# BlaineHeffron/WaveformML

Measured on AMD Instinct MI355X. Metric: waveforms/sec (LitPSD sparse-conv training step), higher is better.
Workload: dtype bf16; 1 GPU; SubMConv3d PSD net, 14x11 PMT grid x 256 samples, Cin=2 Cout=32, 256 events/rank/step, rulebook rebuilt every step; active_voxels_per_rank=84164, global_batch=256, parallelism=dp1, execution=hipgraph

## Files before the change

### include/wfsparse.h

```cpp
#ifndef WFSPARSE_H
#define WFSPARSE_H

#include <stddef.h>
#include <stdint.h>

#ifdef __cplusplus
extern "C" {
#endif

#define WFS_OK 0
#define WFS_EINVAL 1
#define WFS_EOVERFLOW 2
#define WFS_EHIP 3
#define WFS_EWORKSPACE 4

#define WFS_F32 0
#define WFS_BF16 1
#define WFS_F16 2

#define WFS_MAX_DIM 4

#define WFS_ABI_VERSION 6
int wfs_abi_version(void);
const char *wfs_last_error(void);
// ... 188 lines not shown
int wfs_tcnc_ok(int32_t c0, const int32_t *channels, int32_t levels, int32_t k, int32_t L, int32_t dtype);
int wfs_tcnc_n_conv(int32_t c0, const int32_t *channels, int32_t levels, int32_t k);
size_t wfs_tcnc_weights_floats(int32_t c0, const int32_t *channels, int32_t levels, int32_t k);
size_t wfs_tcnc_saved_floats(int64_t N, int32_t L, int32_t c0, const int32_t *channels, int32_t levels);
size_t wfs_tcnc_bwd_workspace_floats(int64_t N, int32_t L, int32_t c0, const int32_t *channels, int32_t levels,
                                     int32_t k);
int wfs_tcnc_taps_fwd(const void *param_ptrs, int32_t c0, const int32_t *channels, int32_t levels, int32_t k,
                      float *wts, void *stream);
int wfs_tcnc_fwd(const void *X, int64_t N, int32_t L, int32_t c0, const int32_t *channels, int32_t levels, int32_t k,
                 const float *wts, float *saved, void *Y, int32_t dtype, float dropout_p, const int64_t *seed_dev,
                 void *stream);
int wfs_tcnc_bwd(const void *X, const void *dY, int64_t N, int32_t L, int32_t c0, const int32_t *channels,
                 int32_t levels, int32_t k, const float *wts, const float *saved, void *dX, float *workspace,
                 const void *param_ptrs, int32_t dtype, float dropout_p, const int64_t *seed_dev, void *stream);

#define WFS_VOXELIZE_MAX_SAMPLES 4096
size_t wfs_voxelize_offsets_ints(int64_t n_cap, int32_t T);
int wfs_voxelize_plan(const void *rows, const int32_t *coords, int64_t n_cap, int32_t T, const int64_t *n_dev,
                      float threshold, int32_t batch_size, int64_t V_cap, int32_t *row_offsets, int64_t *v_dev,
                      int32_t *event_offsets, int32_t *overflow_dev, int32_t dtype, void *stream);
int wfs_voxelize_emit(const void *rows, const void *values, const int32_t *coords, int64_t n_cap, int32_t T,
                      float threshold, const int32_t *row_offsets, int64_t V_cap, int32_t *indices, void *feats,
                      int32_t dtype, void *stream);
int wfs_voxelize_bwd(const void *dfeat, const int32_t *indices, const int32_t *row_offsets, int64_t n_cap, int32_t T,
                     int64_t V_cap, void *dY, int32_t dtype, void *stream);

int wfs_xent_mean_fwd_bwd(const float *logits, const int64_t *target, int64_t B, int32_t C,
                          int64_t ignore_index, float *loss, float *dlogits, void *stream);

int wfs_sgd_step(float *param, const float *grad, float *momentum_buf, int64_t n, const float *lr_dev,
                 float momentum, float dampening, float weight_decay, int32_t nesterov, int32_t first_step,
                 void *stream);

#define WFS_ADAM_COEF_FLOATS 16
int wfs_adam_step(float *param, const float *grad, float *exp_avg, float *exp_avg_sq, float *max_exp_avg_sq,
                  int64_t n, const double *hyper_dev, float *step_dev, float *coef_dev, int32_t amsgrad,
                  int32_t maximize, int32_t decoupled, void *stream);

int wfs_load_batch(const int32_t *coords, int64_t n, int32_t cols, const int32_t *perm_host, int32_t *coords_dst,
                   int32_t *indices_dst, const void *feats, void *feats_dst, int64_t feat_bytes,
                   const int64_t *labels, int64_t *labels_dst, int64_t B, int64_t *n_valid_dst,
                   int32_t *event_offsets, int32_t events, void *stream);

#define WFS_TIMER_GATHER_CONV 0
#define WFS_TIMER_GATHER_DW 1
#define WFS_TIMER_RULEBOOK 2
#define WFS_TIMER_CONV_BACKWARD 3
#define WFS_TIMER_COUNT 4
int wfs_timing_enable(int32_t on);
int wfs_timing_read(int32_t timer, double *total_ms, int64_t *launches);

#ifdef __cplusplus
}
#endif
#endif
```

### waveformml_amd/_lib.py

```python
import ctypes
import os

import torch

_HERE = os.path.dirname(os.path.abspath(__file__))
LIB_PATH = os.environ.get("WFS_LIB") or os.path.join(_HERE, "lib", "libwfsparse.so")

WFS_OK, WFS_EINVAL, WFS_EOVERFLOW, WFS_EHIP, WFS_EWORKSPACE = 0, 1, 2, 3, 4
WFS_F32, WFS_BF16, WFS_F16 = 0, 1, 2
WFS_MAX_DIM = 4
WFS_ABI_VERSION = 6
TIMER_GATHER_CONV, TIMER_GATHER_DW, TIMER_RULEBOOK, TIMER_CONV_BACKWARD = 0, 1, 2, 3

c_i32p = ctypes.POINTER(ctypes.c_int32)
c_i64p = ctypes.POINTER(ctypes.c_int64)
_vp, _i32, _i64, _sz = ctypes.c_void_p, ctypes.c_int32, ctypes.c_int64, ctypes.c_size_t


class Geometry(ctypes.Structure):
    _fields_ = [("ndim", _i32), ("batch_size", _i32), ("subm", _i32), ("K", _i32),
                ("spatial", _i32 * WFS_MAX_DIM), ("out_shape", _i32 * WFS_MAX_DIM),
                ("ksize", _i32 * WFS_MAX_DIM), ("stride", _i32 * WFS_MAX_DIM),
                ("padding", _i32 * WFS_MAX_DIM), ("dilation", _i32 * WFS_MAX_DIM),
                ("transposed", _i32), ("output_padding", _i32 * WFS_MAX_DIM)]
# ... 66 lines not shown
    "wfs_sparse_head_workspace_bytes": (_sz, [_i32, _i64, _i32, _i32]),
    "wfs_sparse_head_fwd": (ctypes.c_int, [_vp, _vp, _vp, _i64, _vp, _i32, _i64, _i32, _vp, _vp, _i32, _vp, _i32, _vp, _sz,
                                           _vp]),
    "wfs_sparse_head_bwd": (ctypes.c_int, [_vp, _vp, _vp, _vp, _i64, _vp, _i32, _i64, _i32, _vp, _i32, _vp, _vp, _vp, _i32,
                                           _vp, _sz, ctypes.POINTER(DwJob), _vp]),
    "wfs_head_workspace_bytes": (_sz, [_i64, _i64, _i32]),
    "wfs_head_fwd": (ctypes.c_int, [_vp, _i64, _i64, _vp, _vp, _i32, _vp, _i32, _vp]),
    "wfs_head_bwd": (ctypes.c_int, [_vp, _vp, _i64, _i64, _vp, _i32, _vp, _vp, _vp, _i32, _vp, _sz, ctypes.POINTER(DwJob),
                                    _vp]),
    "wfs_tcn_lds_bytes": (_sz, [_i32, _i32, _i32]),
    "wfs_tcn_taps_fwd": (ctypes.c_int, [_vp, _i32, _i32, _vp, _vp, _vp]),
    "wfs_tcn_taps_bwd": (ctypes.c_int, [_vp, _i32, _i32, _vp, _i64, _vp]),
    "wfs_tcn_fwd": (ctypes.c_int, [_vp, _i64, _i32, _vp, _vp, _i32, _i32, _vp, _i32, ctypes.c_float, _vp, _vp]),
    "wfs_tcn_bwd": (ctypes.c_int, [_vp, _vp, _i64, _i32, _vp, _vp, _i32, _i32, _vp, _vp, _i32, ctypes.c_float, _vp,
                                    _vp]),
    "wfs_tcnc_ok": (ctypes.c_int, [_i32, c_i32p, _i32, _i32, _i32, _i32]),
    "wfs_tcnc_n_conv": (ctypes.c_int, [_i32, c_i32p, _i32, _i32]),
    "wfs_tcnc_weights_floats": (_sz, [_i32, c_i32p, _i32, _i32]),
    "wfs_tcnc_saved_floats": (_sz, [_i64, _i32, _i32, c_i32p, _i32]),
    "wfs_tcnc_bwd_workspace_floats": (_sz, [_i64, _i32, _i32, c_i32p, _i32, _i32]),
    "wfs_tcnc_taps_fwd": (ctypes.c_int, [_vp, _i32, c_i32p, _i32, _i32, _vp, _vp]),
    "wfs_tcnc_fwd": (ctypes.c_int, [_vp, _i64, _i32, _i32, c_i32p, _i32, _i32, _vp, _vp, _vp, _i32, ctypes.c_float, _vp,
                                    _vp]),
    "wfs_tcnc_bwd": (ctypes.c_int, [_vp, _vp, _i64, _i32, _i32, c_i32p, _i32, _i32, _vp, _vp, _vp, _vp, _vp, _i32,
                                    ctypes.c_float, _vp, _vp]),
    "wfs_voxelize_offsets_ints": (_sz, [_i64, _i32]),
    "wfs_voxelize_plan": (ctypes.c_int, [_vp, _vp, _i64, _i32, _vp, ctypes.c_float, _i32, _i64, _vp, _vp, _vp, _vp, _i32,
                                         _vp]),
    "wfs_voxelize_emit": (ctypes.c_int, [_vp, _vp, _vp, _i64, _i32, ctypes.c_float, _vp, _i64, _vp, _vp, _i32, _vp]),
    "wfs_voxelize_bwd": (ctypes.c_int, [_vp, _vp, _vp, _i64, _i32, _i64, _vp, _i32, _vp]),
    "wfs_xent_mean_fwd_bwd": (ctypes.c_int, [_vp, _vp, _i64, _i32, _i64, _vp, _vp, _vp]),
    "wfs_sgd_step": (ctypes.c_int, [_vp, _vp, _vp, _i64, _vp, ctypes.c_float, ctypes.c_float, ctypes.c_float, _i32, _i32,
                                    _vp]),
    "wfs_adam_step": (ctypes.c_int, [_vp, _vp, _vp, _vp, _vp, _i64, _vp, _vp, _vp, _i32, _i32, _i32, _vp]),
    "wfs_load_batch": (ctypes.c_int, [_vp, _i64, _i32, c_i32p, _vp, _vp, _vp, _vp, _i64, _vp, _vp, _i64, _vp, _vp, _i32,
                                      _vp]),
    "wfs_timing_enable": (ctypes.c_int, [_i32]),
    "wfs_timing_read": (ctypes.c_int, [_i32, ctypes.POINTER(ctypes.c_double), c_i64p]),
}

_LIB = None


def load():
    global _LIB
    if _LIB is None:
        if not os.path.exists(LIB_PATH):
            raise ImportError(
                "libwfsparse.so is missing at %s -- build it with `make -C waveformml_amd/csrc` "
                "(or python -c 'import __graft_entry__ as g; g.build()').  There is no CPU fallback." % LIB_PATH)
        lib = ctypes.CDLL(LIB_PATH)
        for name, (res, args) in SIGNATURES.items():
            fn = getattr(lib, name)
            fn.restype, fn.argtypes = res, args
        got = lib.wfs_abi_version()
        if got != WFS_ABI_VERSION:
            raise ImportError("%s has ABI version %d, this binding was written for %d (struct layouts / signatures "
                              "differ): rebuild with `make -C waveformml_amd/csrc`" % (LIB_PATH, got, WFS_ABI_VERSION))
        wide = os.environ.get("WFS_WIDE_MIN_CHANNELS")
        if wide is not None:
            lib.wfs_wide_enable(int(wide))
        _LIB = lib
    return _LIB


def last_error():
# ... 59 lines not shown
```

### waveformml_amd/csrc/conv_mfma.hip

```cpp
#include <stdlib.h>

#include "wfs_common.h"

namespace {

typedef float f32x16 __attribute__((ext_vector_type(16)));
typedef float f32x4 __attribute__((ext_vector_type(4)));
constexpr int F32_GROUP = 4;

struct KMap {
    int v[128];
};

__device__ __forceinline__ long long valid_rows(long long R, const long long *r_dev) {
    long long v = r_dev ? *r_dev : R;
    return v < R ? v : R;
}

__device__ __forceinline__ int packed_entry(int e, int o) { return (e >= 0 && (e & 7) == o) ? (e >> 3) : -1; }
__device__ __forceinline__ void table_row_of(int pk, int k, int *trow, int *osel) {
    const int kq = pk ? k / pk : k;
    *trow = kq;
    *osel = pk ? k - kq * pk : -1;
}
__device__ __forceinline__ int table_value(int e, int osel) { return osel < 0 ? e : packed_entry(e, osel); }

typedef __bf16 bf16x8e __attribute__((ext_vector_type(8)));
typedef float f32x2 __attribute__((ext_vector_type(2)));

__device__ __forceinline__ void split3_bf16(f32x4 x, bool keep, uint2 &p1, uint2 &p2, uint2 &p3) {
    unsigned u[4], v[4], w[4];
#pragma unroll
    for (int i = 0; i < 4; i += 2) {
        const float xa = x[i], xb = x[i + 1];
        u[i] = keep ? __builtin_bit_cast(unsigned, xa) : 0u;
        u[i + 1] = keep ? __builtin_bit_cast(unsigned, xb) : 0u;
        const f32x2 full = {__builtin_bit_cast(float, u[i]), __builtin_bit_cast(float, u[i + 1])};
        const f32x2 top = {__builtin_bit_cast(float, u[i] & 0xFFFF0000u), __builtin_bit_cast(float, u[i + 1] & 0xFFFF0000u)};
        const f32x2 r = full - top;
        const float ra = r[0], rb = r[1];
        v[i] = __builtin_bit_cast(unsigned, ra);
// ... 485 lines not shown
    const long long Rv = valid_rows(R, r_dev);
    for (long long row = (long long)blockIdx.x * 32 + rsub; row < Rv; row += (long long)gridDim.x * 32) {
        f32x4 acc = bv;
        for (int k = 0; k < K; ++k) {
            int nb = (k == identity_k) ? (int)row : table[(long long)kmap.v[k] * R + row];
            if (nb < 0) continue;
            float x0 = wfs_ld(X + (long long)nb * 2), x1 = wfs_ld(X + (long long)nb * 2 + 1);
            f32x4 w0 = *(const f32x4 *)(sW + k * 64 + cq * 4);
            f32x4 w1 = *(const f32x4 *)(sW + k * 64 + 32 + cq * 4);
            acc.x = fmaf(x0, w0.x, acc.x);
            acc.y = fmaf(x0, w0.y, acc.y);
            acc.z = fmaf(x0, w0.z, acc.z);
            acc.w = fmaf(x0, w0.w, acc.w);
            acc.x = fmaf(x1, w1.x, acc.x);
            acc.y = fmaf(x1, w1.y, acc.y);
            acc.z = fmaf(x1, w1.z, acc.z);
            acc.w = fmaf(x1, w1.w, acc.w);
        }
        T *y = Y + row * 32 + cq * 4;
        if constexpr (sizeof(T) == 4) {
            *reinterpret_cast<f32x4 *>(y) = acc;
        } else {
            uint2 pk;
            pk.x = wfs_pack2<T>(acc.x, acc.y);
            pk.y = wfs_pack2<T>(acc.z, acc.w);
            *reinterpret_cast<uint2 *>(y) = pk;
        }
    }
}

constexpr int DW_KG = 4;
constexpr int DW_WAVES = 8;

constexpr int DW_LDS = DW_WAVES * 1024 * 4;
template <typename T>
__device__ __forceinline__ void gdw32_body(float *sRed, int bx, int by, int nbx, const int *__restrict__ table, int pk, int K,
                                           int identity_k, long long Rcap, const long long *__restrict__ r_dev,
                                           const T *__restrict__ S, const T *__restrict__ G, float *__restrict__ part,
                                           int ngroups) {
    const int lane = threadIdx.x & 63, wid = threadIdx.x >> 6;
    const int j = lane & 31, h = lane >> 5;
    const int g = by;
    const long long R = valid_rows(Rcap, r_dev);
    const long long ntiles = (R + 31) >> 5;
    static_assert(sizeof(T) == 4, "fp32 rows");
    const __amdgpu_buffer_rsrc_t rsrcS = __builtin_amdgcn_make_buffer_rsrc((void *)S, 0, (int)(R * 128), 0x00020000);
    const __amdgpu_buffer_rsrc_t rsrcG = __builtin_amdgcn_make_buffer_rsrc((void *)G, 0, 0x7FFFFFFF, 0x00020000);
    const unsigned j4 = (unsigned)j * 4u;
    f32x16 acc[DW_KG];
#pragma unroll
    for (int q = 0; q < DW_KG; ++q)
#pragma unroll
        for (int i = 0; i < 16; ++i) acc[q][i] = 0.f;
    int trw[DW_KG], osel[DW_KG];
#pragma unroll
    for (int q = 0; q < DW_KG; ++q) {
        const int k = g + q * ngroups;
        table_row_of(pk, k < K ? k : K - 1, &trw[q], &osel[q]);
    }
    for (long long tile = bx + (long long)wid * nbx; tile < ntiles; tile += (long long)DW_WAVES * nbx) {
        const long long row0 = tile * 32;
        const long long trow = row0 + j < R ? row0 + j : R - 1;
        int nbv[DW_KG];
#pragma unroll
        for (int q = 0; q < DW_KG; ++q) nbv[q] = table_value(table[(long long)trw[q] * Rcap + trow], osel[q]);
        float a[16];
        {
// ... 703 lines not shown
    wfs_dw_job j[MAX_DW_JOBS];
    int first[MAX_DW_JOBS + 1];
    int n;
};
__global__ void __launch_bounds__(1024) k_slab_reduce_multi(DwJobs jobs) {
    __shared__ float sR[32][32];
    int ji = 0;
    while (ji + 1 < jobs.n && (int)blockIdx.x >= jobs.first[ji + 1]) ++ji;
    const wfs_dw_job &jb = jobs.j[ji];
    const int nsl = jb.nslabs > 64 ? 32 : 8;
    const int groups = 32 / nsl;
    const int row = threadIdx.x >> 5, lane = threadIdx.x & 31;
    const int grp = row / nsl, sl = row % nsl;
    const long long e = ((long long)((int)blockIdx.x - jobs.first[ji]) * groups + grp) * 32 + lane;
    float s = 0.f;
    if (e < jb.per)
        for (long long c = sl; c < jb.nslabs; c += nsl) s += jb.part[c * jb.per + e];
    sR[row][lane] = s;
    __syncthreads();
    if (sl == 0 && e < jb.per) {
        s = 0.f;
        for (int q = 0; q < nsl; ++q) s += sR[grp * nsl + q][lane];
        if (jb.transpose) {
            const long long ab = (long long)jb.A * jb.B;
            const int k = (int)(e / ab), rem = (int)(e % ab);
            const int a = rem / jb.B, b = rem % jb.B;
            jb.dW[((long long)k * jb.B + b) * jb.A + a] = s;
        } else {
            jb.dW[e] = s;
        }
    }
}

__global__ void __launch_bounds__(1024) k_slab_reduce_multi4(DwJobs jobs) {
    __shared__ f32x4 sR4[32][32];
    int ji = 0;
    while (ji + 1 < jobs.n && (int)blockIdx.x >= jobs.first[ji + 1]) ++ji;
    const wfs_dw_job &jb = jobs.j[ji];
    const int nsl = jb.nslabs > 64 ? 32 : 8;
    const int groups = 32 / nsl;
    const int row = threadIdx.x >> 5, lane = threadIdx.x & 31;
    const int grp = row / nsl, sl = row % nsl;
    const long long e = (((long long)((int)blockIdx.x - jobs.first[ji]) * groups + grp) * 32 + lane) * 4;
    f32x4 s = {0.f, 0.f, 0.f, 0.f};
    if (e < jb.per) {
        constexpr int U = 6;
        for (long long c0 = sl; c0 < jb.nslabs; c0 += (long long)nsl * U) {
            f32x4 v[U];
#pragma unroll
            for (int u = 0; u < U; ++u) {
                const long long c = c0 + (long long)u * nsl;
                const long long cc = c < jb.nslabs ? c : sl;
                v[u] = *(const f32x4 *)(jb.part + cc * jb.per + e);
            }
#pragma unroll
            for (int u = 0; u < U; ++u)
                if (c0 + (long long)u * nsl < jb.nslabs) s += v[u];
        }
    }
    sR4[row][lane] = s;
    __syncthreads();
    if (sl == 0 && e < jb.per) {
        s = f32x4{0.f, 0.f, 0.f, 0.f};
        for (int q = 0; q < nsl; ++q) s += sR4[grp * nsl + q][lane];
        if (jb.transpose) {
            const long long ab = (long long)jb.A * jb.B;
#pragma unroll
            for (int i = 0; i < 4; ++i) {
                const long long ei = e + i;
                const int k = (int)(ei / ab), rem = (int)(ei % ab);
                const int a = rem / jb.B, b = rem % jb.B;
                jb.dW[((long long)k * jb.B + b) * jb.A + a] = s[i];
            }
        } else if ((reinterpret_cast<uintptr_t>(jb.dW + e) & 15) == 0) {
            *(f32x4 *)(jb.dW + e) = s;
        } else {
#pragma unroll
            for (int i = 0; i < 4; ++i) jb.dW[e + i] = s[i];
        }
    }
}

}

int wfs_launch_dw_jobs(const wfs_dw_job *jobs, int n, hipStream_t stream) {
    DwJobs dj;
    dj.n = n;
    bool by4 = true;
    for (int i = 0; i < n; ++i)
        by4 = by4 && jobs[i].per % 4 == 0 && ((uintptr_t)jobs[i].part & 15) == 0;
    int blocks = 0;
    for (int i = 0; i < n; ++i) {
        dj.j[i] = jobs[i];
        dj.first[i] = blocks;
        const long long per_block = (jobs[i].nslabs > 64 ? 32 : 128) * (by4 ? 4 : 1);
        blocks += (int)((jobs[i].per + per_block - 1) / per_block);
    }
    dj.first[n] = blocks;
    if (blocks == 0) return WFS_OK;
    if (by4)
        k_slab_reduce_multi4<<<dim3((unsigned)blocks), dim3(1024), 0, stream>>>(dj);
    else
        k_slab_reduce_multi<<<dim3((unsigned)blocks), dim3(1024), 0, stream>>>(dj);
    WFS_LAUNCH_CHECK();
    return WFS_OK;
}

static bool wfs_split_bf16() {
    static const int on = [] {
        const char *e = getenv("WFS_SPLIT_BF16");
        return (e && e[0] == '0') ? 0 : 1;
    }();
    return on != 0;
}

bool wfs_mfma_gconv32_ok(int K) { return K >= 1 && K <= 32; }

template <typename KernelT, typename... Args>
static int launch_big_lds(KernelT kernel, bool *attr_done, dim3 grid, dim3 block, size_t lds, hipStream_t stream,
                          Args... args) {
    if (!*attr_done) {
        WFS_HIP_CHECK(hipFuncSetAttribute((const void *)kernel, hipFuncAttributeMaxDynamicSharedMemorySize, 158 * 1024));
        *attr_done = true;
    }
    kernel<<<grid, block, lds, stream>>>(args...);
    WFS_LAUNCH_CHECK();
    return WFS_OK;
}

static void gconv32_grid(long long R, bool padded, long long *ntiles, int *wpb, long long *nblk, long long *tiles_per_xcd,
                         int max_waves) {
    *ntiles = (R + 31) >> 5;
    const long long expect = padded ? (*ntiles * 7 + 7) / 8 : *ntiles;
    int w = (int)((expect + 255) / 256);
    w = w < 4 ? 4 : (w > max_waves ? max_waves : (w + 3) / 4 * 4);
    long long nb = (expect + w - 1) / w;
    if (nb > 256) nb = 256;
// ... 311 lines not shown
```

### waveformml_amd/csrc/optim.hip

```cpp
#include "wfs_common.h"

namespace {

__global__ void __launch_bounds__(256) k_sgd_step(float *__restrict__ P, const float *__restrict__ G,
                                                  float *__restrict__ M, long long n, const float *__restrict__ lr_dev,
                                                  float momentum, float dampening, float weight_decay, int nesterov,
                                                  int first_step) {
    const float lr = *lr_dev;
    for (long long i = (long long)blockIdx.x * 256 + threadIdx.x; i < n; i += (long long)gridDim.x * 256) {
        float p = P[i];
        float g = G[i];
        if (weight_decay != 0.f) g = fmaf(weight_decay, p, g);
        if (M) {
            float b = first_step ? g : fmaf(1.f - dampening, g, M[i] * momentum);
            M[i] = b;
            g = nesterov ? fmaf(momentum, b, g) : b;
        }
        P[i] = fmaf(-lr, g, p);
    }
}

}

extern "C" int wfs_sgd_step(float *param, const float *grad, float *momentum_buf, int64_t n, const float *lr_dev,
                            float momentum, float dampening, float weight_decay, int32_t nesterov, int32_t first_step,
                            void *stream_) {
    hipStream_t stream = (hipStream_t)stream_;
    if (n == 0) return WFS_OK;
    WFS_REQUIRE(param && grad && lr_dev, WFS_EINVAL, "NULL device pointer");
    WFS_REQUIRE(momentum_buf || momentum == 0.f, WFS_EINVAL, "momentum needs a buffer");
    long long blocks = wfs_cdiv(n, 256);
    if (blocks > 2048) blocks = 2048;
    k_sgd_step<<<dim3((unsigned)blocks), dim3(256), 0, stream>>>(param, grad, momentum != 0.f ? momentum_buf : nullptr, n,
                                                                 lr_dev, momentum, dampening, weight_decay, nesterov,
                                                                 first_step);
    WFS_LAUNCH_CHECK();
    return WFS_OK;
}

namespace {

struct AdamCoef {
    float decay, wd, w1, omw1, b2, omb2, bc2s, eps, neg_step;
    int has_wd;
};
static_assert(sizeof(AdamCoef) <= WFS_ADAM_COEF_FLOATS * sizeof(float), "coefficient workspace");

__global__ void __launch_bounds__(64) k_adam_prologue(const double *__restrict__ hp, float *__restrict__ step,
                                                      AdamCoef *__restrict__ coef) {
    if (threadIdx.x != 0) return;
    const float t = *step + 1.f;
    *step = t;
    const double lr = hp[0], beta1 = hp[1], beta2 = hp[2], eps = hp[3], wd = hp[4];
    AdamCoef c;
    c.has_wd = wd != 0.0;
    c.decay = (float)(1.0 - lr * wd);
    c.wd = (float)wd;
    c.w1 = (float)(1.0 - beta1);
    c.omw1 = 1.f - c.w1;
    c.b2 = (float)beta2;
    c.omb2 = (float)(1.0 - beta2);
    const double bc1 = 1.0 - pow(beta1, (double)t), bc2 = 1.0 - pow(beta2, (double)t);
    c.bc2s = (float)sqrt(bc2);
    c.eps = (float)eps;
    c.neg_step = (float)(-(lr / bc1));
    *coef = c;
}

template <bool AMS>
__device__ __forceinline__ void adam1(float &p, float g, float &m, float &v, float &vm, const AdamCoef &c, int maximize,
// ... 177 lines not shown
```

### waveformml_amd/csrc/wfs_common.h

```cpp
#pragma once
#include <hip/hip_runtime.h>
#include <stdint.h>
#include <stdio.h>

#include "../../include/wfsparse.h"

#define WFS_WAVE 64

void wfs_set_error(const char *fmt, ...);

#define WFS_HIP_CHECK(expr)                                                                  \
    do {                                                                                     \
        hipError_t _e = (expr);                                                              \
        if (_e != hipSuccess) {                                                              \
            wfs_set_error("%s failed: %s (%s:%d)", #expr, hipGetErrorString(_e), __FILE__,   \
                          __LINE__);                                                         \
            return WFS_EHIP;                                                                 \
        }                                                                                    \
    } while (0)

#define WFS_LAUNCH_CHECK() WFS_HIP_CHECK(hipGetLastError())

#define WFS_REQUIRE(cond, code, ...)                                                         \
    do {                                                                                     \
// ... 30 lines not shown
template <>
__device__ __forceinline__ void wfs_unpack2<wfs_bf16>(unsigned w, float &lo, float &hi) {
    lo = __uint_as_float(w << 16);
    hi = __uint_as_float(w & 0xFFFF0000u);
}
template <>
__device__ __forceinline__ void wfs_unpack2<wfs_f16>(unsigned w, float &lo, float &hi) {
    typedef _Float16 h2 __attribute__((ext_vector_type(2)));
    h2 v = __builtin_bit_cast(h2, w);
    lo = (float)v.x;
    hi = (float)v.y;
}
template <typename H>
__device__ __forceinline__ unsigned wfs_pack2(float lo, float hi);
template <>
__device__ __forceinline__ unsigned wfs_pack2<wfs_bf16>(float lo, float hi) {
    wfs_bf16 a, b;
    wfs_st(&a, lo);
    wfs_st(&b, hi);
    return (unsigned)a | ((unsigned)b << 16);
}
template <>
__device__ __forceinline__ unsigned wfs_pack2<wfs_f16>(float lo, float hi) {
    typedef _Float16 h2 __attribute__((ext_vector_type(2)));
    h2 v = {(_Float16)lo, (_Float16)hi};
    return __builtin_bit_cast(unsigned, v);
}
template <typename H>
__device__ __forceinline__ float wfs_round_to(float v) {
    H t;
    wfs_st(&t, v);
    return wfs_ld(&t);
}
static inline bool wfs_dtype_ok(int dtype) { return dtype == WFS_F32 || dtype == WFS_BF16 || dtype == WFS_F16; }

struct WfsTimerScope {
    int timer;
    hipStream_t stream;
    void *rec;
    WfsTimerScope(int timer, hipStream_t stream);
    ~WfsTimerScope();
};

bool wfs_mfma_gconv32_ok(int K);
int wfs_launch_gconv32_f32(const int *table, int mirror, int K, int identity_k, long long R, const long long *r_dev,
                           const float *X, const float *W, int transpose_w, const float *bias, float *Y,
                           hipStream_t stream, int packed_kl = 0);
int wfs_launch_gconv32_h16(const int *table, int mirror, int K, int identity_k, long long R, const long long *r_dev,
                           const void *X, const float *W, int transpose_w, const float *bias, void *Y, int dtype,
                           hipStream_t stream, int packed_kl = 0);
int wfs_launch_gconv_c2c32(const int *table, const int *kmap, int K, int identity_k, long long R,
                           const long long *r_dev, const void *X, const float *W, const float *bias, void *Y, int dtype,
                           hipStream_t stream);
bool wfs_wide_dw_ok(int K, long long R, int Cs, int Cg, int dtype);
size_t wfs_wide_dw_workspace(int K, long long R, int Cs, int Cg, int dtype);
int wfs_launch_wide_dw(const int *table, const int *kmap_host, int K, int identity_k, long long R, const long long *r_dev,
                       const void *S, int Cs, const void *G, long long G_rows, int Cg, int swap, float *dW, int dtype,
                       void *workspace, size_t workspace_bytes, hipStream_t stream);
size_t wfs_dw_fast_workspace(int K, long long R, int Cs, int Cg);
int wfs_launch_gdw32(const int *table, int K, int identity_k, long long R, const long long *r_dev, const void *S,
                     const void *G, int swap, float *dW, float *part, int dtype, wfs_dw_job *defer, hipStream_t stream,
                     int packed_kl = 0);
bool wfs_bwd32_fused_ok(int K, int packed_kl, int dtype);
int wfs_launch_bwd32_h16(const int *table, int packed_kl, int K, int identity_k, long long R, const long long *r_dev,
                         const void *S, const void *G, const float *W, void *dX, int swap, float *dW, float *part, int dtype,
                         wfs_dw_job *defer, hipStream_t stream);
int wfs_launch_gdw_c32c2(const int *table, int mirror, int K, int identity_k, long long R, const long long *r_dev,
                         const void *S, const void *G, int swap, float *dW, float *part, int dtype,
                         wfs_dw_job *defer, hipStream_t stream);
int wfs_launch_dw_jobs(const wfs_dw_job *jobs, int n, hipStream_t stream);
```

### waveformml_amd/psd/graph.py

```python
import contextlib
import gc
import os
import sys

import torch
import torch.distributed as dist

from .. import _lib
from ..spconv import ops
from .voxel import Voxelizer


@contextlib.contextmanager
def _no_gc():
    was = gc.isenabled()
    gc.disable()
    try:
        yield
    finally:
        if was:
            gc.enable()


def _round_up(v, m):
# ... 150 lines not shown
            return
        _lib.check(_lib.load().wfs_event_offsets(_lib.ptr(self.indices), self.indices.shape[0], self.indices.shape[1] - 1,
                                                 self.n_events, _lib.ptr(self.n_valid), _lib.ptr(self.events),
                                                 _lib.stream_ptr()))


class GraphedTrainStep(_CapturedRunner):
    def __init__(self, module, optimizer, reducer, example_batch, headroom=None, granule=None, warmup=2, min_rows=0):
        (coords, feats), labels = example_batch
        headroom, granule = self._headroom_granule(int(coords.shape[0]), int(labels.shape[0]), headroom, granule)
        assert labels.is_cuda
        per_row = bool(getattr(module, "per_row_targets", False)) and labels.shape[0] == coords.shape[0]
        if per_row:
            self.ignore_index = int(getattr(getattr(module, "criterion", None), "ignore_index", -100))
        net = self._static_buffers(module, example_batch, headroom, granule, min_rows, per_row)
        self.optimizer, self.reducer = optimizer, reducer
        dev = coords.device
        if per_row and net is not None and hasattr(net, "batch_size_hint"):
            net.batch_size_hint = self.n_cap
        if (ops.EVENT_LOCAL and self.indices is not None and 1 <= self.n_events <= ops.EVENT_LOCAL_MAX_BATCH
                and hasattr(net, "batch_events")):
            self.events = torch.zeros((int(_lib.load().wfs_event_offsets_ints(self.n_events)),), dtype=torch.int32,
                                      device=dev)
            net.batch_events = (self.coords, self.events)
        self.world = reducer.world
        exchange = bool(getattr(reducer, "exchange", self.world > 1))
        self.in_graph_exchange = (exchange and dist.is_available() and dist.is_initialized()
                                  and dist.get_backend(reducer.group) == "nccl"
                                  and os.environ.get("WFS_GRAPH_EXCHANGE", "1") != "0")
        if self.in_graph_exchange:
            self.in_graph_exchange = _collective_capture_works(reducer.group, dev)
        self.exchange_after = exchange and not self.in_graph_exchange
        self.in_graph_optimizer = not self.exchange_after and steps_in_graph(optimizer)
        self._own_stream(dev)
        self._fresh_flags()
        reducer.reset()
        loss = module.training_step(([coords, feats], labels), 0)
        loss.backward()
        reducer.finish()
        optimizer.step()
        del loss
        own = _round_up(headroom * coords.shape[0], granule)
        factor = headroom if self.n_cap <= own else self.n_cap / max(1.0, float(coords.shape[0]))
        slack = 1.06 if headroom < 1.05 else 1.0
        self._calibrate(factor, slack, granule)
        if self.exchange_after:
            reducer.remove()
        if self.indices is not None:
            net.batch_first_indices = (self.coords, self.indices)
        self._load(example_batch)
        failed, err = 0, None
        try:
            self._warm_and_capture(warmup)
        except Exception as e:
            if not self.in_graph_exchange:
                raise
            failed, err = 1, e
        if self.in_graph_exchange and self.world > 1:
            failed = _agree_max(failed, reducer.group)
        if failed:
            print("[waveformml_amd] in-graph gradient exchange could not be captured on some rank (%s); exchanging "
                  "after the replay" % (("%s: %s" % (type(err).__name__, err)) if err is not None else "another rank"),
                  file=sys.stderr, flush=True)
            torch.cuda.synchronize()
            self.in_graph_exchange, self.exchange_after, self.in_graph_optimizer = False, True, False
            reducer.remove()
            self._warm_and_capture(warmup)
        self._collect_flags()

    def _warm_and_capture(self, warmup):
        for _ in range(warmup):
            self._body()
            if not self.in_graph_optimizer:
                self._after()
        torch.cuda.synchronize()
        self.graph, self.loss = self._capture(self._body)

    def close(self, remove_hooks=True):
        if self.graph is not None and remove_hooks:
            self.reducer.remove()
        super().close()
        self.loss = None

    def _static_batch(self):
        return ([self.coords, self.feats, self.n_valid], self.labels)

    def _body(self):
        self.reducer.reset()
        from ..spconv import functional as Fsp
        loss = self.module.training_step(self._static_batch(), 0)
        Fsp.defer_dw(self.reducer.flat_param is not None)
        try:
            if loss.dtype == torch.float32 and loss.dim() == 0:
                torch.autograd.backward(loss, grad_tensors=Fsp.unit_loss_grad(loss.device))
            else:
                loss.backward()
            if self.in_graph_exchange:
                self.reducer.finish()
            else:
                self.reducer.pack_all()
        finally:
            Fsp.defer_dw(False)
        if self.in_graph_optimizer:
            self.optimizer.step()
        return loss.detach()

    def _after(self):
        if self.exchange_after:
            self.reducer.exchange_packed()
        self.optimizer.step()

    def eager_step(self, batch):
        self.reducer.reset()
        net = getattr(self.module, "model", None)
        hint = getattr(net, "batch_size_hint", None)
        if self.per_row and hint is not None:
            net.batch_size_hint = None
        try:
            loss = self.module.training_step(batch, 0)
        finally:
            if self.per_row and hint is not None:
                net.batch_size_hint = hint
        loss.backward()
        if self.exchange_after:
            self.reducer.pack_all()
            self.reducer.exchange_packed()
        else:
            self.reducer.finish()
        self.optimizer.step()
        return loss.detach()

    def fits_counts(self, rows_max, labels_min, labels_max, rows_ne_labels):
        if self.per_row:
            return rows_max <= self.n_cap and not rows_ne_labels
        return rows_max <= self.n_cap and labels_min == labels_max == int(self.labels.shape[0])

# ... 190 lines not shown
```

### waveformml_amd/psd/optim.py

```python
import torch

from .. import _lib


class FlatSGD(torch.optim.SGD):
    flat_device_step = True

    def _fast_groups(self):
        for g in self.param_groups:
            ps = g["params"]
            if (len(ps) != 1 or not ps[0].is_cuda or ps[0].dtype != torch.float32 or not ps[0].is_contiguous()
                    or g.get("maximize", False) or g.get("differentiable", False)):
                return False
        return True

    def sync_hyperparameters(self):
        for g in self.param_groups:
            dev = g["params"][0].device
            if g.get("_lr_dev") is None or g["_lr_dev"].device != dev:
                g["_lr_dev"] = torch.empty((1,), dtype=torch.float32, device=dev)
                g["_lr_host"] = None
            if g["_lr_host"] != float(g["lr"]):
                g["_lr_dev"].fill_(float(g["lr"]))
                g["_lr_host"] = float(g["lr"])

    def state_dict(self):
        sd = super().state_dict()
        for g in sd["param_groups"]:
            g.pop("_lr_dev", None)
            g.pop("_lr_host", None)
        sd["state"] = {k: {n: v for n, v in st.items() if n != "_fresh"} for k, st in sd["state"].items()}
        return sd

    def mark_fresh(self):
        for g in self.param_groups:
            if g["dampening"] != 0 and g["momentum"] != 0:
                for p in g["params"]:
                    if "momentum_buffer" in self.state.get(p, {}):
                        self.state[p]["_fresh"] = True

    def has_fresh(self):
        return any(st.get("_fresh", False) for st in self.state.values())

    @torch.no_grad()
    def step(self, closure=None):
        if closure is not None or not self._fast_groups():
            return super().step(closure)
        lib = _lib.load()
        self.sync_hyperparameters()
        for g in self.param_groups:
            p = g["params"][0]
            if p.grad is None:
                continue
            grad = p.grad
            if grad.is_sparse or grad.dtype != torch.float32 or not grad.is_contiguous():
                return super().step(closure)
            state = self.state[p]
            buf, first = state.get("momentum_buffer"), False
            if g["momentum"] != 0 and buf is None:
                buf = state["momentum_buffer"] = torch.empty_like(p, memory_format=torch.contiguous_format)
                first = True
            if state.pop("_fresh", False) and not torch.cuda.is_current_stream_capturing():
                first = True
            _lib.check(lib.wfs_sgd_step(_lib.ptr(p), _lib.ptr(grad), _lib.ptr(buf) if g["momentum"] != 0 else None,
                                        p.numel(), _lib.ptr(g["_lr_dev"]), float(g["momentum"]), float(g["dampening"]),
                                        float(g["weight_decay"]), 1 if g["nesterov"] else 0, 1 if first else 0,
                                        _lib.stream_ptr()))
        return None


_ADAM_COEF_FLOATS = 16


class _FlatAdamStep(object):
    flat_device_step = True

    def _fast_groups(self):
        for g in self.param_groups:
            ps = g["params"]
            if (len(ps) != 1 or not ps[0].is_cuda or ps[0].dtype != torch.float32 or not ps[0].is_contiguous()
                    or torch.is_tensor(g["lr"]) or g.get("differentiable", False)):
                return False
        return True

    @staticmethod
    def _hyper(g):
        beta1, beta2 = g["betas"]
        return (float(g["lr"]), float(beta1), float(beta2), float(g["eps"]), float(g["weight_decay"]))

    def sync_hyperparameters(self):
        dev_blocks = self.__dict__.setdefault("_flat_dev", {})
        capturing = torch.cuda.is_available() and torch.cuda.is_current_stream_capturing()
        for i, g in enumerate(self.param_groups):
            dev = g["params"][0].device
            blk = dev_blocks.get(i)
            if blk is None or blk[0].device != dev:
                if capturing:
                    raise RuntimeError("FlatAdam: the first step runs outside a graph capture (it allocates the "
                                       "hyperparameter block)")
                blk = dev_blocks[i] = [torch.empty((5,), dtype=torch.float64, device=dev),
                                       torch.zeros((_ADAM_COEF_FLOATS,), dtype=torch.float32, device=dev), [None] * 5]
# ... 62 lines not shown
```

### waveformml_amd/spconv/functional.py

```python
import ctypes

import torch
from torch.autograd import Function

from .. import _lib

CONV, SUBM, INVERSE = 0, 1, 2

ACCOUNT = None


def _account(kind, table, R, rows_in, c_in, rows_out, c_out, K, cw_in, cw_out, esize):
    if ACCOUNT is None:
        return
    pairs = int((table >= 0).sum().item()) if table is not None else int(R)
    ACCOUNT.append(dict(kind=kind, pairs=pairs,
                        bytes=rows_in * c_in * esize + rows_out * c_out * esize + pairs * 8 + K * cw_in * cw_out * 4,
                        flops=2 * pairs * cw_in * cw_out))


def _features_ok(t):
    if not t.is_cuda:
        raise RuntimeError("waveformml_amd.spconv: features must be on the GPU (there is no CPU path)")
    return t.contiguous()
# ... 128 lines not shown
            off = param.data_ptr() - fp.data_ptr()
            if 0 <= off and off + 4 * param.numel() <= 4 * fp.numel() and off % 4 == 0:
                slot = fg.data_ptr() + off
                if slot in _SLOTS_WRITTEN:
                    flush_deferred_dw()
                    _SHARED_SLOTS.add(slot)
                    break
                if not _SLOTS_WRITTEN:
                    try:
                        torch.autograd.Variable._execution_engine.queue_callback(reset_grad_slots)
                    except RuntimeError:
                        pass
                _SLOTS_WRITTEN.add(slot)
                return fg[off // 4: off // 4 + param.numel()].view(shape)
    return torch.empty(shape, dtype=torch.float32, device=param.device)


_DEFERRED_DW = None
_DEFERRED_SLOTS = set()
_SHARED_SLOTS = set()


def defer_dw(on):
    global _DEFERRED_DW
    _DEFERRED_DW = [] if on else None
    _DEFERRED_SLOTS.clear()
    _SHARED_SLOTS.clear()


def was_deferred(slot_ptr):
    return slot_ptr in _DEFERRED_SLOTS and slot_ptr not in _SHARED_SLOTS


def flush_deferred_dw():
    if not _DEFERRED_DW:
        return
    lib = _lib.load()
    jobs = (_lib.DwJob * len(_DEFERRED_DW))(*[j for (j, _ws) in _DEFERRED_DW])
    for at in range(0, len(_DEFERRED_DW), 16):
        n = min(16, len(_DEFERRED_DW) - at)
        _lib.check(lib.wfs_dw_reduce_jobs(ctypes.cast(ctypes.byref(jobs, at * ctypes.sizeof(_lib.DwJob)),
                                                      ctypes.POINTER(_lib.DwJob)), n, _lib.stream_ptr()))
    for j, _ws in _DEFERRED_DW:
        _DEFERRED_SLOTS.add(int(j.dW))
    del _DEFERRED_DW[:]


def join_side_streams():
    if _PENDING_SIDE:
        cur = torch.cuda.current_stream()
        for ev, _keep in _PENDING_SIDE:
            cur.wait_event(ev)
        del _PENDING_SIDE[:]


def gather_dw(table, K, identity_k, R, S, G, swap, kmap=None, r_dev=None, overlap=False, like=None, packed_kl=0):
    lib = _lib.load()
    Cs, Cg = int(S.shape[1]), int(G.shape[1])
    shape = (K, Cg, Cs) if swap else (K, Cs, Cg)
    in_slot = False
    if like is not None and like.numel() == K * Cs * Cg:
        dW = grad_like(like, shape)
        in_slot = dW._base is not None
    else:
        dW = torch.empty(shape, dtype=torch.float32, device=S.device)
    assert S.dtype == G.dtype and S.shape[0] == R
    assert table is None or (table.dtype == torch.int32 and table.shape == ((K // packed_kl if packed_kl else K), R))
    nbytes = lib.wfs_gather_dw_workspace_bytes(K, R, Cs, Cg)
    ws = torch.empty((max(int(nbytes), 1),), dtype=torch.uint8, device=S.device)

    def launch():
        defer = _DEFERRED_DW is not None and in_slot and not overlap
        job = _lib.DwJob() if defer else None
        _lib.check(lib.wfs_gather_dw(_lib.ptr(table), kmap, K, identity_k, R, _lib.ptr(S), Cs, _lib.ptr(G), G.shape[0],
                                     Cg, 1 if swap else 0, _lib.ptr(dW), _lib.dtype_code(S), _lib.ptr(ws), ws.numel(),
                                     _lib.ptr(r_dev), ctypes.byref(job) if defer else None, packed_kl, _lib.stream_ptr()))
        if defer and job.nslabs > 0:
            _DEFERRED_DW.append((job, ws))
# ... 613 lines not shown
```

Measured before the change: 559,800 events/s.

## Fuse deferred dW slab reduction with the SGD optimizer step

After: 562,700 events/s, median of 4. No clear change (+0.5%).

```diff
diff --git a/include/wfsparse.h b/include/wfsparse.h
--- a/include/wfsparse.h
+++ b/include/wfsparse.h
@@ -244,6 +244,10 @@
                  float momentum, float dampening, float weight_decay, int32_t nesterov, int32_t first_step,
                  void *stream);
 
+int wfs_dw_reduce_jobs_sgd(const wfs_dw_job *jobs, int32_t n_jobs, float *param, const float *grad,
+                           float *momentum_buf, int64_t n, const float *lr_dev, float momentum, float dampening,
+                           float weight_decay, int32_t nesterov, int32_t first_step, void *stream);
+
 #define WFS_ADAM_COEF_FLOATS 16
 int wfs_adam_step(float *param, const float *grad, float *exp_avg, float *exp_avg_sq, float *max_exp_avg_sq,
                   int64_t n, const double *hyper_dev, float *step_dev, float *coef_dev, int32_t amsgrad,
diff --git a/waveformml_amd/_lib.py b/waveformml_amd/_lib.py
--- a/waveformml_amd/_lib.py
+++ b/waveformml_amd/_lib.py
@@ -122,6 +122,8 @@
     "wfs_xent_mean_fwd_bwd": (ctypes.c_int, [_vp, _vp, _i64, _i32, _i64, _vp, _vp, _vp]),
     "wfs_sgd_step": (ctypes.c_int, [_vp, _vp, _vp, _i64, _vp, ctypes.c_float, ctypes.c_float, ctypes.c_float, _i32, _i32,
                                     _vp]),
+    "wfs_dw_reduce_jobs_sgd": (ctypes.c_int, [ctypes.POINTER(DwJob), _i32, _vp, _vp, _vp, _i64, _vp, ctypes.c_float,
+                                              ctypes.c_float, ctypes.c_float, _i32, _i32, _vp]),
     "wfs_adam_step": (ctypes.c_int, [_vp, _vp, _vp, _vp, _vp, _i64, _vp, _vp, _vp, _i32, _i32, _i32, _vp]),
     "wfs_load_batch": (ctypes.c_int, [_vp, _i64, _i32, c_i32p, _vp, _vp, _vp, _vp, _i64, _vp, _vp, _i64, _vp, _vp, _i32,
                                       _vp]),
diff --git a/waveformml_amd/csrc/conv_mfma.hip b/waveformml_amd/csrc/conv_mfma.hip
--- a/waveformml_amd/csrc/conv_mfma.hip
+++ b/waveformml_amd/csrc/conv_mfma.hip
@@ -6,7 +6,6 @@
 
 typedef float f32x16 __attribute__((ext_vector_type(16)));
 typedef float f32x4 __attribute__((ext_vector_type(4)));
-constexpr int F32_GROUP = 4;
 
 struct KMap {
     int v[128];
@@ -558,7 +557,6 @@
 constexpr int DW_KG = 4;
 constexpr int DW_WAVES = 8;
 
-constexpr int DW_LDS = DW_WAVES * 1024 * 4;
 template <typename T>
 __device__ __forceinline__ void gdw32_body(float *sRed, int bx, int by, int nbx, const int *__restrict__ table, int pk, int K,
                                            int identity_k, long long Rcap, const long long *__restrict__ r_dev,
@@ -1328,8 +1326,35 @@
     }
 }
 
-__global__ void __launch_bounds__(1024) k_slab_reduce_multi4(DwJobs jobs) {
-    __shared__ f32x4 sR4[32][32];
+constexpr int MAX_SGD_RANGES = MAX_DW_JOBS + 1;
+struct SgdTail {
+    wfs_sgd_args a;
+    int nrange;
+    long long start[MAX_SGD_RANGES];
+    long long cum[MAX_SGD_RANGES + 1];
+};
+
+template <bool SGD>
+__device__ __forceinline__ void slab_reduce4(const DwJobs &jobs, const SgdTail &sgd, f32x4 (*sR4)[32]) {
+    float lr = 0.f;
+    if (SGD) {
+        lr = *sgd.a.lr_dev;
+        if ((int)blockIdx.x >= jobs.first[jobs.n]) {
+            const long long total = sgd.cum[sgd.nrange];
+            const long long nth = (long long)((int)gridDim.x - jobs.first[jobs.n]) * 1024;
+            for (long long v = (long long)((int)blockIdx.x - jobs.first[jobs.n]) * 1024 + threadIdx.x; v < total; v += nth) {
+                long long i = v;
+#pragma unroll
+                for (int r = 0; r < MAX_SGD_RANGES; ++r)
+                    if (r < sgd.nrange && v >= sgd.cum[r]) i = sgd.start[r] + (v - sgd.cum[r]);
+                float m = (sgd.a.M && !sgd.a.first_step) ? sgd.a.M[i] : 0.f;
+                sgd.a.P[i] = wfs_sgd1(sgd.a.P[i], sgd.a.G[i], m, sgd.a.M != nullptr, lr, sgd.a.momentum, sgd.a.dampening,
+                                      sgd.a.weight_decay, sgd.a.nesterov, sgd.a.first_step);
+                if (sgd.a.M) sgd.a.M[i] = m;
+            }
+            return;
+        }
+    }
     int ji = 0;
     while (ji + 1 < jobs.n && (int)blockIdx.x >= jobs.first[ji + 1]) ++ji;
     const wfs_dw_job &jb = jobs.j[ji];
@@ -1338,6 +1363,27 @@
     const int row = threadIdx.x >> 5, lane = threadIdx.x & 31;
     const int grp = row / nsl, sl = row % nsl;
     const long long e = (((long long)((int)blockIdx.x - jobs.first[ji]) * groups + grp) * 32 + lane) * 4;
+    const bool writer = sl == 0 && e < jb.per;
+    long long at[4] = {e, e + 1, e + 2, e + 3};
+    if (jb.transpose && writer) {
+        const long long ab = (long long)jb.A * jb.B;
+#pragma unroll
+        for (int i = 0; i < 4; ++i) {
+            const long long ei = e + i;
+            const int k = (int)(ei / ab), rem = (int)(ei % ab);
+            const int a = rem / jb.B, b = rem % jb.B;
+            at[i] = ((long long)k * jb.B + b) * jb.A + a;
+        }
+    }
+    float p[4] = {0.f, 0.f, 0.f, 0.f}, m[4] = {0.f, 0.f, 0.f, 0.f};
+    const long long gi = SGD ? jb.dW - sgd.a.G : 0;
+    if (SGD && writer) {
+#pragma unroll
+        for (int i = 0; i < 4; ++i) {
+            p[i] = sgd.a.P[gi + at[i]];
+            if (sgd.a.M && !sgd.a.first_step) m[i] = sgd.a.M[gi + at[i]];
+        }
+    }
     f32x4 s = {0.f, 0.f, 0.f, 0.f};
     if (e < jb.per) {
         constexpr int U = 6;
@@ -1356,35 +1402,41 @@
     }
     sR4[row][lane] = s;
     __syncthreads();
-    if (sl == 0 && e < jb.per) {
+    if (writer) {
         s = f32x4{0.f, 0.f, 0.f, 0.f};
         for (int q = 0; q < nsl; ++q) s += sR4[grp * nsl + q][lane];
         if (jb.transpose) {
-            const long long ab = (long long)jb.A * jb.B;
-#pragma unroll
-            for (int i = 0; i < 4; ++i) {
-                const long long ei = e + i;
-                const int k = (int)(ei / ab), rem = (int)(ei % ab);
-                const int a = rem / jb.B, b = rem % jb.B;
-                jb.dW[((long long)k * jb.B + b) * jb.A + a] = s[i];
-            }
+#pragma unroll
+            for (int i = 0; i < 4; ++i) jb.dW[at[i]] = s[i];
         } else if ((reinterpret_cast<uintptr_t>(jb.dW + e) & 15) == 0) {
             *(f32x4 *)(jb.dW + e) = s;
         } else {
 #pragma unroll
             for (int i = 0; i < 4; ++i) jb.dW[e + i] = s[i];
         }
-    }
-}
-
-}
-
-int wfs_launch_dw_jobs(const wfs_dw_job *jobs, int n, hipStream_t stream) {
-    DwJobs dj;
+        if (SGD) {
+#pragma unroll
+            for (int i = 0; i < 4; ++i) {
+                sgd.a.P[gi + at[i]] = wfs_sgd1(p[i], s[i], m[i], sgd.a.M != nullptr, lr, sgd.a.momentum, sgd.a.dampening,
+                                               sgd.a.weight_decay, sgd.a.nesterov, sgd.a.first_step);
+                if (sgd.a.M) sgd.a.M[gi + at[i]] = m[i];
+            }
+        }
+    }
+}
+
+__global__ void __launch_bounds__(1024) k_slab_reduce_multi4(DwJobs jobs) {
+    __shared__ f32x4 sR4[32][32];
+    slab_reduce4<false>(jobs, SgdTail{}, sR4);
+}
+
+__global__ void __launch_bounds__(1024, 8) k_slab_reduce_sgd4(DwJobs jobs, SgdTail sgd) {
+    __shared__ f32x4 sR4[32][32];
+    slab_reduce4<true>(jobs, sgd, sR4);
+}
+
+int dw_job_blocks(const wfs_dw_job *jobs, int n, bool by4, DwJobs &dj) {
     dj.n = n;
-    bool by4 = true;
-    for (int i = 0; i < n; ++i)
-        by4 = by4 && jobs[i].per % 4 == 0 && ((uintptr_t)jobs[i].part & 15) == 0;
     int blocks = 0;
     for (int i = 0; i < n; ++i) {
         dj.j[i] = jobs[i];
@@ -1393,12 +1445,74 @@
         blocks += (int)((jobs[i].per + per_block - 1) / per_block);
     }
     dj.first[n] = blocks;
+    return blocks;
+}
+
+bool dw_jobs_by4(const wfs_dw_job *jobs, int n) {
+    bool by4 = true;
+    for (int i = 0; i < n; ++i)
+        by4 = by4 && jobs[i].per % 4 == 0 && ((uintptr_t)jobs[i].part & 15) == 0;
+    return by4;
+}
+
+}
+
+int wfs_launch_dw_jobs(const wfs_dw_job *jobs, int n, hipStream_t stream) {
+    DwJobs dj;
+    const bool by4 = dw_jobs_by4(jobs, n);
+    const int blocks = dw_job_blocks(jobs, n, by4, dj);
     if (blocks == 0) return WFS_OK;
     if (by4)
         k_slab_reduce_multi4<<<dim3((unsigned)blocks), dim3(1024), 0, stream>>>(dj);
     else
         k_slab_reduce_multi<<<dim3((unsigned)blocks), dim3(1024), 0, stream>>>(dj);
     WFS_LAUNCH_CHECK();
+    return WFS_OK;
+}
+
+int wfs_launch_dw_jobs_sgd(const wfs_dw_job *jobs, int n, const wfs_sgd_args &sgd, int *fused, hipStream_t stream) {
+    *fused = 0;
+    if (n < 1 || n > MAX_DW_JOBS || sgd.n <= 0 || !dw_jobs_by4(jobs, n)) return WFS_OK;
+    long long lo[MAX_DW_JOBS], hi[MAX_DW_JOBS];
+    for (int i = 0; i < n; ++i) {
+        const uintptr_t d = (uintptr_t)jobs[i].dW, g = (uintptr_t)sgd.G;
+        if (d < g || (d - g) % sizeof(float) != 0) return WFS_OK;
+        const long long o = (long long)((d - g) / sizeof(float));
+        if (o + jobs[i].per > sgd.n) return WFS_OK;
+        if (jobs[i].transpose && jobs[i].per != (long long)jobs[i].K * jobs[i].A * jobs[i].B) return WFS_OK;
+        int at = i;
+        for (; at > 0 && lo[at - 1] > o; --at) {
+            lo[at] = lo[at - 1];
+            hi[at] = hi[at - 1];
+        }
+        lo[at] = o;
+        hi[at] = o + jobs[i].per;
+    }
+    for (int i = 1; i < n; ++i)
+        if (lo[i] < hi[i - 1]) return WFS_OK;
+    SgdTail t;
+    t.a = sgd;
+    t.nrange = 0;
+    long long total = 0, from = 0;
+    for (int i = 0; i <= n; ++i) {
+        const long long to = i < n ? lo[i] : sgd.n;
+        if (to > from) {
+            t.start[t.nrange] = from;
+            t.cum[t.nrange] = total;
+            total += to - from;
+            ++t.nrange;
+        }
+        if (i < n) from = hi[i];
+    }
+    for (int r = t.nrange; r <= MAX_SGD_RANGES; ++r) t.cum[r] = total;
+    for (int r = t.nrange; r < MAX_SGD_RANGES; ++r) t.start[r] = 0;
+    DwJobs dj;
+    const int blocks = dw_job_blocks(jobs, n, true, dj);
+    long long extra = (total + 1023) / 1024;
+    if (extra > 256) extra = 256;
+    k_slab_reduce_sgd4<<<dim3((unsigned)(blocks + extra)), dim3(1024), 0, stream>>>(dj, t);
+    WFS_LAUNCH_CHECK();
+    *fused = 1;
     return WFS_OK;
 }
 
diff --git a/waveformml_amd/csrc/optim.hip b/waveformml_amd/csrc/optim.hip
--- a/waveformml_amd/csrc/optim.hip
+++ b/waveformml_amd/csrc/optim.hip
@@ -8,15 +8,9 @@
                                                   int first_step) {
     const float lr = *lr_dev;
     for (long long i = (long long)blockIdx.x * 256 + threadIdx.x; i < n; i += (long long)gridDim.x * 256) {
-        float p = P[i];
-        float g = G[i];
-        if (weight_decay != 0.f) g = fmaf(weight_decay, p, g);
-        if (M) {
-            float b = first_step ? g : fmaf(1.f - dampening, g, M[i] * momentum);
-            M[i] = b;
-            g = nesterov ? fmaf(momentum, b, g) : b;
-        }
-        P[i] = fmaf(-lr, g, p);
+        float m = (M && !first_step) ? M[i] : 0.f;
+        P[i] = wfs_sgd1(P[i], G[i], m, M != nullptr, lr, momentum, dampening, weight_decay, nesterov, first_step);
+        if (M) M[i] = m;
     }
 }
 
@@ -36,6 +30,40 @@
                                                                  first_step);
     WFS_LAUNCH_CHECK();
     return WFS_OK;
+}
+
+extern "C" int wfs_dw_reduce_jobs_sgd(const wfs_dw_job *jobs, int32_t n, float *param, const float *grad,
+                                      float *momentum_buf, int64_t numel, const float *lr_dev, float momentum,
+                                      float dampening, float weight_decay, int32_t nesterov, int32_t first_step,
+                                      void *stream_) {
+    hipStream_t stream = (hipStream_t)stream_;
+    WFS_REQUIRE(n >= 0 && n <= 16 && (n == 0 || jobs), WFS_EINVAL, "%d jobs (0 .. 16)", n);
+    WFS_REQUIRE(numel >= 0, WFS_EINVAL, "negative size");
+    WFS_REQUIRE(numel == 0 || (param && grad && lr_dev), WFS_EINVAL, "NULL device pointer");
+    WFS_REQUIRE(momentum_buf || momentum == 0.f, WFS_EINVAL, "momentum needs a buffer");
+    wfs_dw_job live[16];
+    int m = 0;
+    for (int i = 0; i < n; ++i) {
+        if (jobs[i].nslabs <= 0) continue;
+        WFS_REQUIRE(jobs[i].part && jobs[i].dW && jobs[i].per > 0 && jobs[i].A > 0 && jobs[i].B > 0, WFS_EINVAL,
+                    "job %d is incomplete", i);
+        live[m++] = jobs[i];
+    }
+    if (m > 0 && numel > 0) {
+        const wfs_sgd_args sgd = {param, grad, momentum != 0.f ? momentum_buf : nullptr, numel, lr_dev, momentum,
+                                  dampening, weight_decay, nesterov, first_step};
+        int fused = 0;
+        WfsTimerScope timer(WFS_TIMER_GATHER_DW, stream);
+        const int rc = wfs_launch_dw_jobs_sgd(live, m, sgd, &fused, stream);
+        if (rc != WFS_OK || fused) return rc;
+    }
+    if (m > 0) {
+        WfsTimerScope timer(WFS_TIMER_GATHER_DW, stream);
+        const int rc = wfs_launch_dw_jobs(live, m, stream);
+        if (rc != WFS_OK) return rc;
+    }
+    return wfs_sgd_step(param, grad, momentum_buf, numel, lr_dev, momentum, dampening, weight_decay, nesterov, first_step,
+                        stream_);
 }
 
 namespace {
diff --git a/waveformml_amd/csrc/wfs_common.h b/waveformml_amd/csrc/wfs_common.h
--- a/waveformml_amd/csrc/wfs_common.h
+++ b/waveformml_amd/csrc/wfs_common.h
@@ -86,6 +86,15 @@
     wfs_st(&t, v);
     return wfs_ld(&t);
 }
+__device__ __forceinline__ float wfs_sgd1(float p, float g, float &m, bool has_m, float lr, float momentum,
+                                          float dampening, float weight_decay, int nesterov, int first_step) {
+    if (weight_decay != 0.f) g = fmaf(weight_decay, p, g);
+    if (has_m) {
+        m = first_step ? g : fmaf(1.f - dampening, g, m * momentum);
+        g = nesterov ? fmaf(momentum, m, g) : m;
+    }
+    return fmaf(-lr, g, p);
+}
 static inline bool wfs_dtype_ok(int dtype) { return dtype == WFS_F32 || dtype == WFS_BF16 || dtype == WFS_F16; }
 
 struct WfsTimerScope {
@@ -123,3 +132,13 @@
                          const void *S, const void *G, int swap, float *dW, float *part, int dtype,
                          wfs_dw_job *defer, hipStream_t stream);
 int wfs_launch_dw_jobs(const wfs_dw_job *jobs, int n, hipStream_t stream);
+struct wfs_sgd_args {
+    float *P;
+    const float *G;
+    float *M;
+    long long n;
+    const float *lr_dev;
+    float momentum, dampening, weight_decay;
+    int nesterov, first_step;
+};
+int wfs_launch_dw_jobs_sgd(const wfs_dw_job *jobs, int n, const wfs_sgd_args &sgd, int *fused, hipStream_t stream);
diff --git a/waveformml_amd/psd/graph.py b/waveformml_amd/psd/graph.py
--- a/waveformml_amd/psd/graph.py
+++ b/waveformml_amd/psd/graph.py
@@ -206,6 +206,8 @@
             self.in_graph_exchange = _collective_capture_works(reducer.group, dev)
         self.exchange_after = exchange and not self.in_graph_exchange
         self.in_graph_optimizer = not self.exchange_after and steps_in_graph(optimizer)
+        from .optim import fused_tail_ok
+        self.fused_tail = self.in_graph_optimizer and not exchange and fused_tail_ok(optimizer, reducer)
         self._own_stream(dev)
         self._fresh_flags()
         reducer.reset()
@@ -238,6 +240,7 @@
                   file=sys.stderr, flush=True)
             torch.cuda.synchronize()
             self.in_graph_exchange, self.exchange_after, self.in_graph_optimizer = False, True, False
+            self.fused_tail = False
             reducer.remove()
             self._warm_and_capture(warmup)
         self._collect_flags()
@@ -269,13 +272,16 @@
                 torch.autograd.backward(loss, grad_tensors=Fsp.unit_loss_grad(loss.device))
             else:
                 loss.backward()
+            pending = Fsp.take_deferred_dw() if self.fused_tail else None
             if self.in_graph_exchange:
                 self.reducer.finish()
             else:
                 self.reducer.pack_all()
         finally:
             Fsp.defer_dw(False)
-        if self.in_graph_optimizer:
+        if self.fused_tail:
+            self.optimizer.step(reduce_jobs=pending)
+        elif self.in_graph_optimizer:
             self.optimizer.step()
         return loss.detach()
 
diff --git a/waveformml_amd/psd/optim.py b/waveformml_amd/psd/optim.py
--- a/waveformml_amd/psd/optim.py
+++ b/waveformml_amd/psd/optim.py
@@ -1,3 +1,5 @@
+import os
+
 import torch
 
 from .. import _lib
@@ -43,17 +45,27 @@
         return any(st.get("_fresh", False) for st in self.state.values())
 
     @torch.no_grad()
-    def step(self, closure=None):
+    def step(self, closure=None, reduce_jobs=None):
+        from ..spconv import functional as Fsp
+        fuse = reduce_jobs is not None and len(self.param_groups) == 1
+        if reduce_jobs and not fuse:
+            Fsp.reduce_dw_jobs(reduce_jobs)
         if closure is not None or not self._fast_groups():
+            if fuse:
+                Fsp.reduce_dw_jobs(reduce_jobs)
             return super().step(closure)
         lib = _lib.load()
         self.sync_hyperparameters()
         for g in self.param_groups:
             p = g["params"][0]
             if p.grad is None:
+                if fuse:
+                    Fsp.reduce_dw_jobs(reduce_jobs)
                 continue
             grad = p.grad
             if grad.is_sparse or grad.dtype != torch.float32 or not grad.is_contiguous():
+                if fuse:
+                    Fsp.reduce_dw_jobs(reduce_jobs)
                 return super().step(closure)
             state = self.state[p]
             buf, first = state.get("momentum_buffer"), False
@@ -62,11 +74,29 @@
                 first = True
             if state.pop("_fresh", False) and not torch.cuda.is_current_stream_capturing():
                 first = True
-            _lib.check(lib.wfs_sgd_step(_lib.ptr(p), _lib.ptr(grad), _lib.ptr(buf) if g["momentum"] != 0 else None,
-                                        p.numel(), _lib.ptr(g["_lr_dev"]), float(g["momentum"]), float(g["dampening"]),
-                                        float(g["weight_decay"]), 1 if g["nesterov"] else 0, 1 if first else 0,
-                                        _lib.stream_ptr()))
+            args = (_lib.ptr(p), _lib.ptr(grad), _lib.ptr(buf) if g["momentum"] != 0 else None, p.numel(),
+                    _lib.ptr(g["_lr_dev"]), float(g["momentum"]), float(g["dampening"]), float(g["weight_decay"]),
+                    1 if g["nesterov"] else 0, 1 if first else 0)
+            if fuse:
+                Fsp.reduce_dw_jobs(reduce_jobs, sgd=args)
+            else:
+                _lib.check(lib.wfs_sgd_step(*(args + (_lib.stream_ptr(),))))
         return None
+
+
+def fused_tail_ok(optimizer, reducer):
+    if os.environ.get("WFS_FUSE_TAIL", "1") == "0":
+        return False
+    if not isinstance(optimizer, FlatSGD) or type(optimizer).step is not FlatSGD.step:
+        return False
+    if bool(getattr(reducer, "exchange", getattr(reducer, "world", 1) > 1)) or getattr(reducer, "world", 1) > 1:
+        return False
+    flat = getattr(reducer, "flat_param", None)
+    if flat is None or len(optimizer.param_groups) != 1:
+        return False
+    params = optimizer.param_groups[0]["params"]
+    return (len(params) == 1 and params[0] is flat and flat.grad is reducer.flat_grad and flat.is_contiguous()
+            and reducer.flat_grad.is_contiguous() and flat.dtype == torch.float32)
 
 
 _ADAM_COEF_FLOATS = 16
diff --git a/waveformml_amd/spconv/functional.py b/waveformml_amd/spconv/functional.py
--- a/waveformml_amd/spconv/functional.py
+++ b/waveformml_amd/spconv/functional.py
@@ -184,18 +184,33 @@
     return slot_ptr in _DEFERRED_SLOTS and slot_ptr not in _SHARED_SLOTS
 
 
-def flush_deferred_dw():
+def reduce_dw_jobs(pending, sgd=None):
+    if not pending and sgd is None:
+        return
+    lib = _lib.load()
+    jobs = (_lib.DwJob * max(len(pending), 1))(*[j for (j, _ws) in pending])
+    last = max(0, (len(pending) - 1) // 16 * 16)
+    for at in range(0, max(len(pending), 1), 16):
+        n = min(16, len(pending) - at)
+        some = ctypes.cast(ctypes.byref(jobs, at * ctypes.sizeof(_lib.DwJob)), ctypes.POINTER(_lib.DwJob))
+        if sgd is not None and at == last:
+            _lib.check(lib.wfs_dw_reduce_jobs_sgd(some, n, *(tuple(sgd) + (_lib.stream_ptr(),))))
+        else:
+            _lib.check(lib.wfs_dw_reduce_jobs(some, n, _lib.stream_ptr()))
+
+
+def take_deferred_dw():
     if not _DEFERRED_DW:
-        return
-    lib = _lib.load()
-    jobs = (_lib.DwJob * len(_DEFERRED_DW))(*[j for (j, _ws) in _DEFERRED_DW])
-    for at in range(0, len(_DEFERRED_DW), 16):
-        n = min(16, len(_DEFERRED_DW) - at)
-        _lib.check(lib.wfs_dw_reduce_jobs(ctypes.cast(ctypes.byref(jobs, at * ctypes.sizeof(_lib.DwJob)),
-                                                      ctypes.POINTER(_lib.DwJob)), n, _lib.stream_ptr()))
-    for j, _ws in _DEFERRED_DW:
+        return []
+    taken = list(_DEFERRED_DW)
+    for j, _ws in taken:
         _DEFERRED_SLOTS.add(int(j.dW))
     del _DEFERRED_DW[:]
+    return taken
+
+
+def flush_deferred_dw():
+    reduce_dw_jobs(take_deferred_dw())
 
 
 def join_side_streams():
```
